# KerkDovan/univer-ocr

Measured on NVIDIA B200. Metric: my_model inference images/sec (page tiles through Monochrome->Paragraph + Line + Char forward), higher is better.
Workload: dtype tf32/f32

## Files before the change

### univer_ocr_b200/csrc/tc_gemm.cu

```cuda
#include <cuda.h>

#include <mutex>

#include "conv_common.cuh"
#include "gemm_common.cuh"
#include "tc_ptx.cuh"

namespace uocr {

typedef CUresult (*EncodeTiledFn)(CUtensorMap*, CUtensorMapDataType, cuuint32_t, void*, const cuuint64_t*,
                                  const cuuint64_t*, const cuuint32_t*, const cuuint32_t*,
                                  CUtensorMapInterleave, CUtensorMapSwizzle, CUtensorMapL2promotion,
                                  CUtensorMapFloatOOBfill);

static EncodeTiledFn encode_tiled() {
    static EncodeTiledFn fn = nullptr;
    static std::once_flag once;
    std::call_once(once, [] {
        void* p = nullptr;
        cudaDriverEntryPointQueryResult q;
        if (cudaGetDriverEntryPoint("cuTensorMapEncodeTiled", &p, cudaEnableDefault, &q) == cudaSuccess &&
            q == cudaDriverEntryPointSuccess)
            fn = reinterpret_cast<EncodeTiledFn>(p);
    });
// ... 603 lines not shown
        const uint64_t da[2] = {(uint64_t)K, (uint64_t)M}, sa[1] = {(uint64_t)lda * 4};
        const uint32_t ba[2] = {TC_BK, TC_BM};
        rc = make_tmap(&ma, A, 2, da, sa, ba);
    }
    if (rc) return rc;
    const uint64_t db[2] = {(uint64_t)K, (uint64_t)N}, sb[1] = {(uint64_t)ldb * 4};
    const uint32_t bb[2] = {TC_BK, (uint32_t)(pair ? p.nt / 2 : p.nt)};
    rc = make_tmap(&mb, Bt, 2, db, sb, bb);
    if (rc) return rc;
    static int num_sms = 0, num_pairs = 0;
    if (!num_sms) {
        int dev = 0;
        cudaGetDevice(&dev);
        cudaDeviceGetAttribute(&num_sms, cudaDevAttrMultiProcessorCount, dev);
        cudaError_t e = cudaFuncSetAttribute(tc_gemm_persistent_kernel<false>, cudaFuncAttributeMaxDynamicSharedMemorySize,
                                             227 * 1024);
        if (e == cudaSuccess)
            e = cudaFuncSetAttribute(tc_gemm_persistent_kernel<true>, cudaFuncAttributeMaxDynamicSharedMemorySize,
                                     227 * 1024);
        if (e != cudaSuccess) { num_sms = 0; set_error("cudaFuncSetAttribute: %s", cudaGetErrorString(e)); return UOCR_ERR_CUDA; }
    }
    const int n_tiles = (int)ceil_div(N, p.nt);
    if (pair) {
        const int m_tiles = (int)ceil_div(M, 2 * TC_BM);
        const int64_t tiles = (int64_t)m_tiles * n_tiles;
        cudaLaunchConfig_t cfg{};
        cudaLaunchAttribute attr[1];
        attr[0].id = cudaLaunchAttributeClusterDimension;
        attr[0].val.clusterDim.x = 2; attr[0].val.clusterDim.y = 1; attr[0].val.clusterDim.z = 1;
        cfg.blockDim = dim3(TCP_THREADS); cfg.dynamicSmemBytes = smem; cfg.stream = st; cfg.attrs = attr; cfg.numAttrs = 1;
        if (!num_pairs) {
            cfg.gridDim = dim3((unsigned)num_sms & ~1u);
            int n = 0;
            if (cudaOccupancyMaxActiveClusters(&n, tc_gemm_persistent_kernel<true>, &cfg) != cudaSuccess || n <= 0) {
                cudaGetLastError();
                n = num_sms / 2;
            }
            num_pairs = n < num_sms / 2 ? n : num_sms / 2;
        }
        cfg.gridDim = dim3(2u * (unsigned)(tiles < num_pairs ? tiles : num_pairs));
        cudaError_t e = cudaLaunchKernelEx(&cfg, tc_gemm_persistent_kernel<true>, ma, mb, p, m_tiles, n_tiles);
        if (e != cudaSuccess) { set_error("cluster launch: %s", cudaGetErrorString(e)); return UOCR_ERR_CUDA; }
        UOCR_LAUNCHED("tc_gemm_persistent_pair_tf32");
        return UOCR_OK;
    }
    const int m_tiles = (int)ceil_div(M, TC_BM);
    const int64_t tiles = (int64_t)m_tiles * n_tiles;
    const unsigned grid = (unsigned)(tiles < num_sms ? tiles : num_sms);
    tc_gemm_persistent_kernel<false><<<grid, TCP_THREADS, smem, st>>>(ma, mb, p, m_tiles, n_tiles);
    UOCR_LAUNCHED("tc_gemm_persistent_tf32");
    return UOCR_OK;
}

int tc_gemm_mn_atomic(const float* At, int64_t lda, const float* B, int64_t ldb, float* C, int64_t ldc,
                      int64_t M, int64_t N, int64_t K, cudaStream_t st) {
    if ((lda % 4) || (ldb % 4) || ((reinterpret_cast<uintptr_t>(At) | reinterpret_cast<uintptr_t>(B)) & 15))
        return UOCR_ERR_UNSUPPORTED;
    if (M <= 0 || N <= 0 || K <= 0 || M > 0x7fffffff || K > 0x7fffffff) return UOCR_ERR_UNSUPPORTED;
    TcParams p{};
    p.C = C; p.ldc = ldc; p.M = M; p.N = N; p.num_kb = (int)ceil_div(K, TC_BK);
    p.nt = N >= 256 ? 256 : (int)(((N + 31) / 32) * 32);
    p.act = UOCR_ACT_NONE; p.atomic = 1;
    const int64_t tiles = ceil_div(M, TC_BM) * ceil_div(N, p.nt);
    int64_t splits = (148 + tiles - 1) / tiles;
    if (splits > p.num_kb / 8) splits = p.num_kb / 8;
    if (splits < 1) splits = 1;
    if (splits > 65535) splits = 65535;
    p.kb_per_split = (int)ceil_div(p.num_kb, splits);
    splits = ceil_div(p.num_kb, p.kb_per_split);
    CUtensorMap ma, mb;
    const uint64_t da[2] = {(uint64_t)M, (uint64_t)K}, sa[1] = {(uint64_t)lda * 4};
    const uint32_t box[2] = {32, TC_BK};
    int rc = make_tmap(&ma, At, 2, da, sa, box, true);
    if (rc) return rc;
    const uint64_t db[2] = {(uint64_t)N, (uint64_t)K}, sb[1] = {(uint64_t)ldb * 4};
    rc = make_tmap(&mb, B, 2, db, sb, box, true);
    if (rc) return rc;
    dim3 grid((unsigned)ceil_div(M, TC_BM), (unsigned)ceil_div(N, p.nt), (unsigned)splits);
    return launch_tc<TC_GEMM_MN>(ma, mb, p, grid, st);
}

__global__ void __launch_bounds__(256) transpose_kernel(const float* __restrict__ src, float* __restrict__ dst,
                                                        int rows, int cols, int64_t src_pitch, int64_t dst_pitch) {
    __shared__ float t[32][33];
    const int c0 = blockIdx.x * 32, r0 = blockIdx.y * 32;
    const int tx = threadIdx.x & 31, ty = threadIdx.x >> 5;
    for (int i = ty; i < 32; i += 8) {
        const int r = r0 + i, c = c0 + tx;
        t[i][tx] = (r < rows && c < cols) ? src[(int64_t)r * src_pitch + c] : 0.f;
    }
    __syncthreads();
    for (int i = ty; i < 32; i += 8) {
        const int c = c0 + i, r = r0 + tx;
        if (c < cols && r < rows) dst[(int64_t)c * dst_pitch + r] = t[tx][i];
    }
}

static int transpose_async(const float* src, float* dst, int rows, int cols, int64_t src_pitch, int64_t dst_pitch,
                           cudaStream_t st) {
    dim3 grid((cols + 31) / 32, (rows + 31) / 32);
    transpose_kernel<<<grid, 256, 0, st>>>(src, dst, rows, cols, src_pitch, dst_pitch);
    UOCR_LAUNCHED("transpose");
    return UOCR_OK;
}

int fc_fwd_fast(int math_mode, const float* x, const float* w, const float* w_kmajor, float* y, int64_t batch,
                int64_t n_in, int64_t n_out, int act, float alpha, cudaStream_t st) {
    if (math_mode != UOCR_MATH_TF32) return UOCR_ERR_UNSUPPORTED;
    if (n_in % 4 || batch < 128 || n_in < 32 || n_out < 16) return UOCR_ERR_UNSUPPORTED;
    if (!encode_tiled()) return UOCR_ERR_UNSUPPORTED;
    Scratch wt(st);
    if (!w_kmajor) {
        int rc = wt.alloc(sizeof(float) * n_out * n_in);
        if (rc) return rc;
        rc = transpose_async(w, (float*)wt.ptr, (int)n_in, (int)n_out, n_out, n_in, st);
        if (rc) return rc;
        w_kmajor = (const float*)wt.ptr;
    }
    return tc_gemm_tn(x, n_in, w_kmajor, n_in, y, n_out, batch, n_out, n_in, w + n_in * n_out, act, alpha, 0, st);
}

int fc_window_fwd_fast(int math_mode, const float* x, const float* w, const float* w_kmajor, float* y, int64_t n,
                       int64_t wd, int64_t c, int width, int64_t n_out, int act, float alpha, cudaStream_t st) {
    const int64_t n_in = (int64_t)width * c, batch = n * wd;
    if (math_mode != UOCR_MATH_TF32 || !encode_tiled()) return UOCR_ERR_UNSUPPORTED;
    if (wd % TC_BM || c % TC_BK || n_out < 128 || n_out % 4 || (reinterpret_cast<uintptr_t>(x) & 15)) return UOCR_ERR_UNSUPPORTED;
    const int64_t nt = n_out >= 256 ? 256 : ((n_out + 15) / 16) * 16;
    if (ceil_div(batch, TC_BM) * ceil_div(n_out, nt) < 96) return UOCR_ERR_UNSUPPORTED;
    Scratch wt(st);
    if (!w_kmajor) {
        int rc = wt.alloc(sizeof(float) * n_out * n_in);
        if (rc) return rc;
        rc = transpose_async(w, (float*)wt.ptr, (int)n_in, (int)n_out, n_out, n_in, st);
        if (rc) return rc;
        w_kmajor = (const float*)wt.ptr;
    }
    const WindowGeom win{n, wd, c, width};
    return tc_gemm_tn_persistent_impl(x, 0, &win, w_kmajor, n_in, y, n_out, batch, n_out, n_in, w + n_in * n_out, act,
                                      alpha, 0, st);
}

int weights_to_kmajor(const float* w, float* wt, int64_t k_rows, int64_t n_cols, cudaStream_t st) {
    if (k_rows > 0x7fffffff || n_cols > 0x7fffffff) return UOCR_ERR_UNSUPPORTED;
    return transpose_async(w, wt, (int)k_rows, (int)n_cols, n_cols, k_rows, st);
}

__global__ void __launch_bounds__(256) colsum_kernel(const float* __restrict__ src, int64_t rows, int cols,
                                                     int64_t rows_per_block, float* __restrict__ out) {
    __shared__ float red[8][33];
    const int c = blockIdx.x * 32 + (threadIdx.x & 31);
    const int ty = threadIdx.x >> 5;
    const int64_t r0 = (int64_t)blockIdx.y * rows_per_block;
    const int64_t r1 = min(rows, r0 + rows_per_block);
    float s0 = 0.f, s1 = 0.f, s2 = 0.f, s3 = 0.f;
    if (c < cols) {
        int64_t r = r0 + ty;
        for (; r + 24 < r1; r += 32) {
            s0 += __ldg(src + r * cols + c);
            s1 += __ldg(src + (r + 8) * cols + c);
            s2 += __ldg(src + (r + 16) * cols + c);
            s3 += __ldg(src + (r + 24) * cols + c);
        }
        for (; r < r1; r += 8) s0 += __ldg(src + r * cols + c);
    }
    red[ty][threadIdx.x & 31] = (s0 + s1) + (s2 + s3);
    __syncthreads();
    if (ty == 0 && c < cols) {
        float t = 0.f;
#pragma unroll
        for (int k = 0; k < 8; ++k) t += red[k][threadIdx.x];
        atomicAdd(out + c, t);
    }
}

static int colsum_async(const float* src, int64_t rows, int cols, float* out, int accumulate, cudaStream_t st) {
    if (!accumulate) {
        cudaError_t e = cudaMemsetAsync(out, 0, sizeof(float) * cols, st);
        if (e != cudaSuccess) { set_error("memset: %s", cudaGetErrorString(e)); return UOCR_ERR_CUDA; }
    }
    const int gx = (cols + 31) / 32;
    int64_t gy = ceil_div(148 * 8, gx);
    const int64_t max_gy = ceil_div(rows, 64);
    if (gy > max_gy) gy = max_gy;
    if (gy < 1) gy = 1;
    if (gy > 65535) gy = 65535;
    const int64_t rpb = ceil_div(rows, gy);
    colsum_kernel<<<dim3((unsigned)gx, (unsigned)ceil_div(rows, rpb)), 256, 0, st>>>(src, rows, cols, rpb, out);
    UOCR_LAUNCHED("colsum");
    return UOCR_OK;
// ... 534 lines not shown
```

### univer_ocr_b200/csrc/hourglass.cu

```cuda
#include "conv_common.cuh"
#include "tc_ptx.cuh"

namespace uocr {

struct HourglassParams {
    const float* x; float* y;
    const float* w[5]; const float* b[5];
    int H, W;
    float alpha;
    int act_end; float alpha_end;
};

constexpr int HG_WSLOT = 28;

template <int TH, int TW>
struct HG {
    static constexpr int XH = TH + 25, XW = TW + 27, XP = (XW + 1 + 3) & ~3, XROWS = XH + 2;
    static constexpr int D1H = TH / 2 + 11, D1W = TW / 2 + 11, D1P = (D1W + 3 + 3) & ~3;
    static constexpr int D2H = TH / 4 + 4, D2W = TW / 4 + 4, D2P = (D2W + 2 + 3 + 3) & ~3;
    static constexpr int U2H = TH / 2 + 4, U2W = TW / 2 + 4, U2P = (U2W + 3 + 3) & ~3;
    static constexpr int U1H = TH + 4, U1W = TW + 4, U1P = (U1W + 3 + 3) & ~3;
    static constexpr int FLOATS = XROWS * XP + D1H * D1P + D2H * D2P + U2H * U2P + 5 * HG_WSLOT + 2 * 36 + 6;
    static_assert(U1H * U1P <= XROWS * XP, "U1 fits into the x block");
};

constexpr int HG_THREADS = 256;
__host__ __device__ constexpr int hg_threads(int th) { return th >= 64 ? 512 : HG_THREADS; }

template <int N4>
__device__ __forceinline__ void hg_load_weights(const float* __restrict__ src, float* w) {
#pragma unroll
    for (int i = 0; i < N4; ++i) {
        const float4 v = reinterpret_cast<const float4*>(src)[i];
        w[4 * i] = v.x; w[4 * i + 1] = v.y; w[4 * i + 2] = v.z; w[4 * i + 3] = v.w;
    }
}

template <int DH, int DW, int DP, int SP, int R, int NT>
__device__ __forceinline__ void hg_down(const float* __restrict__ src, float* __restrict__ dst, const float* __restrict__ wb,
                                        int gy0, int gx0, int hl, int wl, float alpha) {
    float w[28];
    hg_load_weights<7>(wb, w);
    const float bias = w[25];
    constexpr int STRIPS = (DH + R - 1) / R;
    for (int item = threadIdx.x; item < STRIPS * DW; item += NT) {
        const int s = item / DW, c = item - s * DW, r0 = R * s;
        float acc[R];
#pragma unroll
        for (int j = 0; j < R; ++j) acc[j] = bias;
#pragma unroll
        for (int rr = 0; rr < 2 * R + 3; ++rr) {
            const float2* row = reinterpret_cast<const float2*>(src + (2 * r0 + rr) * SP + 2 * c);
            const float2 a = row[0], b = row[1], e = row[2];
            const float in[5] = {a.x, a.y, b.x, b.y, e.x};
#pragma unroll
            for (int j = 0; j < R; ++j) {
                const int ky = rr - 2 * j;
                if (ky >= 0 && ky < 5) {
#pragma unroll
                    for (int kx = 0; kx < 5; ++kx) acc[j] = fmaf(w[ky * 5 + kx], in[kx], acc[j]);
                }
            }
        }
        const bool colin = (unsigned)(gx0 + c) < (unsigned)wl;
#pragma unroll
        for (int j = 0; j < R; ++j) {
            const float v = fmaxf(acc[j], acc[j] * alpha);
            if (r0 + j < DH) dst[(r0 + j) * DP + c] = (colin && (unsigned)(gy0 + r0 + j) < (unsigned)hl) ? v : 0.f;
        }
    }
}

template <int DH, int DW, int DP, int SP, int R, int NT>
__device__ __forceinline__ void hg_down_pairs(const float* __restrict__ src, float* __restrict__ dst, const float* __restrict__ wb,
                                              int gy0, int gx0, int hl, int wl, float alpha) {
    float w[28];
    hg_load_weights<7>(wb, w);
    const float bias = w[25];
    constexpr int STRIPS = (DH + R - 1) / R, PAIRS = DW / 2 + 1;
    for (int item = threadIdx.x; item < STRIPS * PAIRS; item += NT) {
        const int s = item / PAIRS, pr = item - s * PAIRS, r0 = R * s;
        float acc[R][2];
#pragma unroll
        for (int j = 0; j < R; ++j) acc[j][0] = acc[j][1] = bias;
#pragma unroll
        for (int rr = 0; rr < 2 * R + 3; ++rr) {
            const float4* row = reinterpret_cast<const float4*>(src + (2 * r0 + rr) * SP + 4 * pr);
            const float4 u = row[0], v = row[1];
            const float in[8] = {u.x, u.y, u.z, u.w, v.x, v.y, v.z, v.w};
#pragma unroll
            for (int j = 0; j < R; ++j) {
                const int ky = rr - 2 * j;
                if (ky >= 0 && ky < 5) {
#pragma unroll
                    for (int kx = 0; kx < 5; ++kx) {
                        acc[j][0] = fmaf(w[ky * 5 + kx], in[kx], acc[j][0]);
                        acc[j][1] = fmaf(w[ky * 5 + kx], in[2 + kx], acc[j][1]);
                    }
                }
            }
        }
        const int c1 = 2 * pr, c0 = c1 - 1;
        const bool in0 = pr > 0 && (unsigned)(gx0 + c0) < (unsigned)wl, in1 = c1 < DW && (unsigned)(gx0 + c1) < (unsigned)wl;
#pragma unroll
        for (int j = 0; j < R; ++j) {
            if (r0 + j < DH) {
                const bool rowin = (unsigned)(gy0 + r0 + j) < (unsigned)hl;
                const float v0 = fmaxf(acc[j][0], acc[j][0] * alpha), v1 = fmaxf(acc[j][1], acc[j][1] * alpha);
                if (pr > 0) dst[(r0 + j) * DP + c0] = (rowin && in0) ? v0 : 0.f;
                if (c1 < DW) dst[(r0 + j) * DP + c1] = (rowin && in1) ? v1 : 0.f;
            }
        }
    }
}

template <int DH, int DW, int DP, int SP, int NT>
__device__ __forceinline__ void hg_up(const float* __restrict__ src, float* __restrict__ dst, const float* __restrict__ wf,
                                      float bias, int gy0, int gx0, int hl, int wl, float alpha) {
    float w[36];
    hg_load_weights<9>(wf, w);
    constexpr int GROUPS = (DW + 3) / 4;
    for (int item = threadIdx.x; item < (DH / 2) * GROUPS; item += NT) {
        const int j = item / GROUPS, n0 = (item - j * GROUPS) * 2;
        float s[3][4];
#pragma unroll
        for (int a = 0; a < 3; ++a) {
            const float2* row = reinterpret_cast<const float2*>(src + (j + a) * SP + n0);
            const float2 u = row[0], v = row[1];
            s[a][0] = u.x; s[a][1] = u.y; s[a][2] = v.x; s[a][3] = v.y;
        }
#pragma unroll
        for (int py = 0; py < 2; ++py) {
            float o[4];
#pragma unroll
            for (int i = 0; i < 2; ++i)
#pragma unroll
                for (int px = 0; px < 2; ++px) {
                    float acc = bias;
#pragma unroll
                    for (int a = 0; a < 3; ++a)
#pragma unroll
                        for (int b = 0; b < 3; ++b) acc = fmaf(w[((py * 2 + px) * 3 + a) * 3 + b], s[a][i + b], acc);
                    o[2 * i + px] = fmaxf(acc, acc * alpha);
                }
            const bool rowin = (unsigned)(gy0 + 2 * j + py) < (unsigned)hl;
#pragma unroll
            for (int k = 0; k < 4; ++k)
                if (!(rowin && (unsigned)(gx0 + 2 * n0 + k) < (unsigned)wl)) o[k] = 0.f;
            *reinterpret_cast<float4*>(dst + (2 * j + py) * DP + 2 * n0) = make_float4(o[0], o[1], o[2], o[3]);
        }
    }
}

template <int NT>
__device__ __forceinline__ void hg_fold(const float* __restrict__ w25, float* __restrict__ wf) {
    for (int i = threadIdx.x; i < 36; i += NT) {
        const int b = i % 3, a = (i / 3) % 3, px = (i / 9) % 2, py = i / 18;
        const int ylo = py == 0 ? 2 * a : (a == 0 ? 0 : 2 * a - 1), yhi = py == 0 ? min(2 * a + 1, 4) : (a == 0 ? 0 : 2 * a);
        const int xlo = px == 0 ? 2 * b : (b == 0 ? 0 : 2 * b - 1), xhi = px == 0 ? min(2 * b + 1, 4) : (b == 0 ? 0 : 2 * b);
        float s = 0.f;
        for (int ky = ylo; ky <= yhi; ++ky)
            for (int kx = xlo; kx <= xhi; ++kx) s += w25[ky * 5 + kx];
        wf[i] = s;
    }
}

template <int TH, int TW>
__global__ void __launch_bounds__(hg_threads(TH), TH >= 64 ? 2 : 4) hourglass1_fwd_kernel(const HourglassParams p,
                                                                       const __grid_constant__ CUtensorMap map_x) {
    using G = HG<TH, TW>;
    constexpr int NT = hg_threads(TH);
    extern __shared__ __align__(128) float hg_smem[];
    float* sX = hg_smem;
    float* sD1 = sX + G::XROWS * G::XP;
    float* sD2 = sD1 + G::D1H * G::D1P;
    float* sU2 = sD2 + G::D2H * G::D2P;
    float* sU1 = sX;
    float* sW = sU2 + G::U2H * G::U2P;
    float* sF = sW + 5 * HG_WSLOT;

    const int ox0 = blockIdx.x * TW, oy0 = blockIdx.y * TH;
    float* yim = p.y + (int64_t)blockIdx.z * p.H * p.W;
    const int tid = threadIdx.x;

    uint64_t* bar = reinterpret_cast<uint64_t*>(sF + 2 * 36);
    if (tid == 0) {
        mbar_init(smem_u32(bar), 1);
        asm volatile("fence.mbarrier_init.release.cluster;" ::: "memory");
        mbar_arrive_expect_tx(smem_u32(bar), (uint32_t)(G::XH * G::XP * sizeof(float)));
        tma_load_3d(smem_u32(sX), &map_x, smem_u32(bar), ox0 - 16, oy0 - 14, (int)blockIdx.z);
    }
    if (tid < 26) {
#pragma unroll
        for (int l = 0; l < 5; ++l) sW[l * HG_WSLOT + tid] = tid < 25 ? __ldg(p.w[l] + tid) : __ldg(p.b[l]);
    }
    for (int i = tid; i < 2 * G::XP; i += NT) sX[G::XH * G::XP + i] = 0.f;
    __syncthreads();
    mbar_wait(smem_u32(bar), 0);
    hg_fold<NT>(sW + 2 * HG_WSLOT, sF);
    hg_fold<NT>(sW + 3 * HG_WSLOT, sF + 36);
    const int hy0 = oy0 / 2, hx0 = ox0 / 2, qy0 = oy0 / 4, qx0 = ox0 / 4;
    hg_down_pairs<G::D1H, G::D1W, G::D1P, G::XP, 5, NT>(sX, sD1, sW, hy0 - 6, hx0 - 6, p.H / 2, p.W / 2, p.alpha);
    __syncthreads();
    hg_down<G::D2H, G::D2W, G::D2P, G::D1P, (G::D2H % 2 == 0) ? 2 : 4, NT>(sD1, sD2, sW + HG_WSLOT, qy0 - 2, qx0 - 2, p.H / 4, p.W / 4, p.alpha);
    __syncthreads();
    hg_up<G::U2H, G::U2W, G::U2P, G::D2P, NT>(sD2, sU2, sF, sW[2 * HG_WSLOT + 25], hy0 - 2, hx0 - 2, p.H / 2, p.W / 2, p.alpha);
    __syncthreads();
    hg_up<G::U1H, G::U1W, G::U1P, G::U2P, NT>(sU2, sU1, sF + 36, sW[3 * HG_WSLOT + 25], oy0 - 2, ox0 - 2, p.H, p.W, p.alpha);
    __syncthreads();
    {
        float w[28];
        hg_load_weights<7>(sW + 4 * HG_WSLOT, w);
        const float bias = w[25];
        constexpr int GROUPS = TW / 4, RE = 4;
        for (int item = tid; item < (TH / RE) * GROUPS; item += NT) {
            const int r = (item / GROUPS) * RE, c0 = (item - (item / GROUPS) * GROUPS) * 4;
            float acc[RE][4];
#pragma unroll
            for (int k = 0; k < RE; ++k)
#pragma unroll
                for (int j = 0; j < 4; ++j) acc[k][j] = bias;
#pragma unroll
            for (int rr = 0; rr < RE + 4; ++rr) {
                const float4* row = reinterpret_cast<const float4*>(sU1 + (r + rr) * G::U1P + c0);
                const float4 u = row[0], v = row[1];
                const float in[8] = {u.x, u.y, u.z, u.w, v.x, v.y, v.z, v.w};
#pragma unroll
                for (int k = 0; k < RE; ++k) {
                    const int ky = rr - k;
                    if (ky >= 0 && ky < 5) {
#pragma unroll
                        for (int kx = 0; kx < 5; ++kx)
#pragma unroll
                            for (int j = 0; j < 4; ++j) acc[k][j] = fmaf(w[ky * 5 + kx], in[j + kx], acc[k][j]);
                    }
                }
            }
            const int gx = ox0 + c0;
            if (gx < p.W) {
#pragma unroll
                for (int k = 0; k < RE; ++k) {
                    const int gy = oy0 + r + k;
                    if (gy < p.H)
                        *reinterpret_cast<float4*>(yim + (int64_t)gy * p.W + gx) =
                            make_float4(apply_act_fast(acc[k][0], p.act_end, p.alpha_end),
                                        apply_act_fast(acc[k][1], p.act_end, p.alpha_end),
                                        apply_act_fast(acc[k][2], p.act_end, p.alpha_end),
                                        apply_act_fast(acc[k][3], p.act_end, p.alpha_end));
                }
            }
        }
    }
}

static int hourglass1_unsupported() {
    set_error("hourglass1_fwd: unsupported geometry (H, W must be multiples of 4)");
    return UOCR_ERR_UNSUPPORTED;
}

template <int TH>
static int hourglass1_launch(const HourglassParams& p, const float* x, int64_t n, int64_t h, int64_t wd, cudaStream_t st) {
    constexpr int TW = 128;
    using G = HG<TH, TW>;
    const uint64_t dims[3] = {(uint64_t)wd, (uint64_t)h, (uint64_t)n};
    const uint64_t strides[2] = {(uint64_t)wd * 4, (uint64_t)wd * h * 4};
    const uint32_t box[3] = {(uint32_t)G::XP, (uint32_t)G::XH, 1};
    CUtensorMap map{};
    const int rc = make_tmap_plain_f32(&map, x, 3, dims, strides, box);
    if (rc != UOCR_OK) return rc;
    const size_t smem = sizeof(float) * G::FLOATS;
    static bool configured = false;
    if (!configured) {
        cudaError_t e = cudaFuncSetAttribute(hourglass1_fwd_kernel<TH, TW>, cudaFuncAttributeMaxDynamicSharedMemorySize,
                                             (int)smem);
        if (e != cudaSuccess) { set_error("cudaFuncSetAttribute: %s", cudaGetErrorString(e)); return UOCR_ERR_CUDA; }
        configured = true;
    }
    dim3 grid((unsigned)ceil_div(wd, TW), (unsigned)ceil_div(h, TH), (unsigned)n);
    if (grid.y > 65535) return hourglass1_unsupported();
    hourglass1_fwd_kernel<TH, TW><<<grid, hg_threads(TH), smem, st>>>(p, map);
    UOCR_LAUNCHED("hourglass1_fwd");
    return UOCR_OK;
}

int hourglass1_fwd(const float* x, const float* const* w, const float* const* b, float* y, int64_t n, int64_t h,
                   int64_t wd, float alpha, int act_end, float alpha_end, cudaStream_t st) {
    if (h % 4 || wd % 4 || n > 65535 || alpha < 0.f || alpha > 1.f) return hourglass1_unsupported();
    if ((reinterpret_cast<uintptr_t>(x) | reinterpret_cast<uintptr_t>(y)) & 15) return hourglass1_unsupported();
    HourglassParams p{};
    p.x = x; p.y = y;
    for (int l = 0; l < 5; ++l) { p.w[l] = w[l]; p.b[l] = b[l]; }
    p.H = (int)h; p.W = (int)wd; p.alpha = alpha; p.act_end = act_end; p.alpha_end = alpha_end;
    const int64_t blocks64 = n * ceil_div(h, 64) * ceil_div(wd, 128);
    if (blocks64 >= 148 * 2 * 2) return hourglass1_launch<64>(p, x, n, h, wd, st);
    return hourglass1_launch<32>(p, x, n, h, wd, st);
}

}

static int hourglass1_entry(const float* x, const float* const* weights, const float* const* biases, float* y, int64_t n,
                            int64_t h, int64_t w, float alpha, int act_end, float alpha_end, int math_mode, void* stream) {
    using namespace uocr;
    UOCR_REQUIRE(x && y && weights && biases, "NULL pointer");
    for (int l = 0; l < 5; ++l) UOCR_REQUIRE(weights[l] && biases[l], "NULL weight pointer (level %d)", l);
    UOCR_REQUIRE(n > 0 && h > 0 && w > 0 && h < (1 << 30) && w < (1 << 30), "bad dimension");
    UOCR_REQUIRE(act_end >= UOCR_ACT_NONE && act_end <= UOCR_ACT_SIGMOID, "unknown activation %d", act_end);
    UOCR_REQUIRE(math_mode == UOCR_MATH_FP32 || math_mode == UOCR_MATH_TF32, "unknown math mode %d", math_mode);
    return hourglass1_fwd(x, weights, biases, y, n, h, w, alpha, act_end, alpha_end, as_stream(stream));
}

extern "C" int uocr_hourglass1_fwd(const float* x, const float* const* weights, const float* const* biases, float* y,
                                   int64_t n, int64_t h, int64_t w, float alpha, int act_end, float alpha_end,
                                   void* stream) {
    return hourglass1_entry(x, weights, biases, y, n, h, w, alpha, act_end, alpha_end, UOCR_MATH_FP32, stream);
}

extern "C" int uocr_hourglass1_fwd_mode(const float* x, const float* const* weights, const float* const* biases, float* y,
                                        int64_t n, int64_t h, int64_t w, float alpha, int act_end, float alpha_end,
                                        int math_mode, void* stream) {
    return hourglass1_entry(x, weights, biases, y, n, h, w, alpha, act_end, alpha_end, math_mode, stream);
}
```

Baseline: 171,600.

## Add slab-reuse tcgen05 kernel for sliding-window FC layers

After: 173,700 (median of 6 runs). +1.2%, better.

```diff
diff --git a/univer_ocr_b200/csrc/tc_gemm.cu b/univer_ocr_b200/csrc/tc_gemm.cu
--- a/univer_ocr_b200/csrc/tc_gemm.cu
+++ b/univer_ocr_b200/csrc/tc_gemm.cu
@@ -679,6 +679,260 @@
     return UOCR_OK;
 }
 
+constexpr int WFC_CHUNK = 128;
+constexpr uint32_t WFC_HALF_BYTES = WFC_CHUNK * TC_BK * 4;
+
+struct WinFcParams {
+    float* y; int64_t n_out;
+    int m_tiles, n_tiles;
+    int chunks_per_row;
+    int64_t chunks;
+    int tiles_per_line;
+    int cblocks, half, num_kb;
+    int rot_period;
+    int stages;
+    uint32_t slab_bytes, slab_box_bytes;
+    int act; float alpha;
+};
+
+struct WinFcUnits {
+    int64_t q, end;
+    int cpr;
+    __device__ WinFcUnits(const WinFcParams& p)
+        : q(p.chunks * blockIdx.x / gridDim.x), end(p.chunks * (blockIdx.x + 1) / gridDim.x), cpr(p.chunks_per_row) {}
+    __device__ bool next(int& mt, int& col0, int& ncols) {
+        if (q >= end) return false;
+        mt = (int)(q / cpr);
+        const int cq = (int)(q - (int64_t)mt * cpr);
+        const bool two = (cq & 1) == 0 && q + 1 < end;
+        col0 = cq * WFC_CHUNK; ncols = two ? 2 * WFC_CHUNK : WFC_CHUNK;
+        q += two ? 2 : 1;
+        return true;
+    }
+};
+
+__global__ void __launch_bounds__(TCP_THREADS, 1) tc_window_fc_kernel(const __grid_constant__ CUtensorMap map_x,
+                                                                     const __grid_constant__ CUtensorMap map_b,
+                                                                     const float* __restrict__ bias, const WinFcParams p) {
+    extern __shared__ __align__(1024) uint8_t smem_raw[];
+    uint8_t* smem = reinterpret_cast<uint8_t*>((reinterpret_cast<uintptr_t>(smem_raw) + 1023) & ~(uintptr_t)1023);
+    const uint32_t slab_set = (uint32_t)p.cblocks * p.slab_bytes;
+    constexpr uint32_t stage_bytes = 2 * WFC_HALF_BYTES;
+    uint8_t* slab = smem;
+    uint8_t* ring = smem + 2 * slab_set;
+    float* s_bias = reinterpret_cast<float*>(ring + (size_t)p.stages * stage_bytes);
+    float* s_stage = s_bias + p.n_out;
+    uint64_t* bars = reinterpret_cast<uint64_t*>(s_stage + 8 * 512);
+    uint64_t* full = bars;
+    uint64_t* empty = bars + p.stages;
+    uint64_t* tmem_full = bars + 2 * p.stages;
+    uint64_t* tmem_empty = bars + 2 * p.stages + 2;
+    uint64_t* slab_full = bars + 2 * p.stages + 4;
+    uint64_t* slab_empty = bars + 2 * p.stages + 6;
+    uint32_t* tmem_slot = reinterpret_cast<uint32_t*>(bars + 2 * p.stages + 8);
+
+    const int warp = threadIdx.x >> 5, lane = threadIdx.x & 31;
+    for (int i = threadIdx.x; i < p.n_out; i += TCP_THREADS) s_bias[i] = bias ? __ldg(bias + i) : 0.f;
+    if (threadIdx.x == 0) {
+        for (int s = 0; s < p.stages; ++s) {
+            mbar_init(smem_u32(&full[s]), 1);
+            mbar_init(smem_u32(&empty[s]), 1);
+        }
+        for (int b = 0; b < 2; ++b) {
+            mbar_init(smem_u32(&tmem_full[b]), 1);
+            mbar_init(smem_u32(&tmem_empty[b]), 8);
+            mbar_init(smem_u32(&slab_full[b]), 1);
+            mbar_init(smem_u32(&slab_empty[b]), 1);
+        }
+        asm volatile("fence.mbarrier_init.release.cluster;" ::: "memory");
+    }
+    if (warp == 1) {
+        asm volatile("tcgen05.alloc.cta_group::1.sync.aligned.shared::cta.b32 [%0], %1;"
+                     ::"r"(smem_u32(tmem_slot)), "r"(4 * WFC_CHUNK) : "memory");
+        asm volatile("tcgen05.relinquish_alloc_permit.cta_group::1.sync.aligned;" ::: "memory");
+    }
+    tc_fence_before();
+    __syncthreads();
+    tc_fence_after();
+    const uint32_t tmem_base = *tmem_slot;
+    auto first_kb = [&](int mt, int col0) {
+        return p.rot_period ? (int)(((int64_t)mt * p.n_tiles + col0 / (2 * WFC_CHUNK)) % p.rot_period) % p.num_kb : 0;
+    };
+
+    if (warp == 0) {
+        if (lane == 0) {
+            WinFcUnits units(p);
+            int it = 0, r = -1, cur = -1, mt, col0, ncols;
+            while (units.next(mt, col0, ncols)) {
+                if (mt != cur) {
+                    cur = mt; ++r;
+                    const int buf = r & 1;
+                    const int line = mt / p.tiles_per_line, wx0 = (mt - line * p.tiles_per_line) * TC_BM;
+                    mbar_wait(smem_u32(&slab_empty[buf]), ((r >> 1) & 1) ^ 1);
+                    mbar_arrive_expect_tx(smem_u32(&slab_full[buf]), (uint32_t)p.cblocks * p.slab_box_bytes);
+                    for (int cb = 0; cb < p.cblocks; ++cb)
+                        tma_load_3d(smem_u32(slab + buf * slab_set + cb * p.slab_bytes), &map_x,
+                                    smem_u32(&slab_full[buf]), cb * TC_BK, wx0 - p.half, line);
+                }
+                const int rot = first_kb(mt, col0);
+                for (int kb = 0; kb < p.num_kb; ++kb, ++it) {
+                    const int s = it % p.stages;
+                    mbar_wait(smem_u32(&empty[s]), ((it / p.stages) & 1) ^ 1);
+                    const int kbr = kb + rot >= p.num_kb ? kb + rot - p.num_kb : kb + rot;
+                    const uint32_t sb = smem_u32(ring + s * stage_bytes);
+                    mbar_arrive_expect_tx(smem_u32(&full[s]), (uint32_t)ncols * TC_BK * 4);
+                    for (int h = 0; h < ncols; h += WFC_CHUNK)
+                        tma_load_2d(sb + (uint32_t)h * TC_BK * 4, &map_b, smem_u32(&full[s]), kbr * TC_BK, col0 + h);
+                }
+            }
+        }
+    } else if (warp == 1) {
+        if (lane == 0) {
+            const uint32_t idesc0 = (1u << 4) | (2u << 7) | (2u << 10) | ((uint32_t)(TC_BM >> 4) << 24);
+            WinFcUnits units(p);
+            int it = 0, t = 0, r = -1, cur = -1, mt, col0, ncols;
+            uint32_t slab0 = 0;
+            while (units.next(mt, col0, ncols)) {
+                if (mt != cur) {
+                    if (r >= 0) tc_commit(smem_u32(&slab_empty[r & 1]));
+                    cur = mt; ++r;
+                    mbar_wait(smem_u32(&slab_full[r & 1]), (r >> 1) & 1);
+                    tc_fence_after();
+                    slab0 = smem_u32(slab + (r & 1) * slab_set);
+                }
+                const int acc = t & 1;
+                mbar_wait(smem_u32(&tmem_empty[acc]), ((t >> 1) & 1) ^ 1);
+                tc_fence_after();
+                const uint32_t tacc = tmem_base + (uint32_t)(acc * 2 * WFC_CHUNK);
+                const uint32_t idesc = idesc0 | ((uint32_t)(ncols >> 3) << 17);
+                const int rot = first_kb(mt, col0);
+                for (int kb = 0; kb < p.num_kb; ++kb, ++it) {
+                    const int s = it % p.stages;
+                    mbar_wait(smem_u32(&full[s]), (it / p.stages) & 1);
+                    tc_fence_after();
+                    const int kbr = kb + rot >= p.num_kb ? kb + rot - p.num_kb : kb + rot;
+                    const int k = kbr / p.cblocks, cb = kbr - k * p.cblocks;
+                    const uint64_t da = make_kmajor_sw128_desc(slab0 + (uint32_t)cb * p.slab_bytes + (uint32_t)k * 128u);
+                    const uint64_t db = make_kmajor_sw128_desc(smem_u32(ring + s * stage_bytes));
+#pragma unroll
+                    for (int kk = 0; kk < TC_BK / 8; ++kk)
+                        tc_mma_tf32(tacc, da + (uint64_t)(kk * 2), db + (uint64_t)(kk * 2), idesc,
+                                    (kb > 0 || kk > 0) ? 1u : 0u);
+                    tc_commit(smem_u32(&empty[s]));
+                }
+                tc_commit(smem_u32(&tmem_full[acc]));
+                ++t;
+            }
+        }
+    } else {
+        const int e = warp - 2, q = warp & 3, half = e >> 2;
+        float4* stg = reinterpret_cast<float4*>(s_stage) + e * 128;
+        const int sub_r = lane >> 2, sub_g = lane & 3;
+        WinFcUnits units(p);
+        int t = 0, mt, col0, ncols;
+        while (units.next(mt, col0, ncols)) {
+            const int acc = t & 1;
+            const int nhc = ncols >> 4;
+            float* yrow = p.y + ((int64_t)mt * TC_BM + q * 32) * p.n_out;
+            mbar_wait(smem_u32(&tmem_full[acc]), (t >> 1) & 1);
+            tc_fence_after();
+            const uint32_t tq = tmem_base + ((uint32_t)(q * 32) << 16) + (uint32_t)(acc * 2 * WFC_CHUNK);
+            uint32_t va[16], vb[16];
+            auto handle = [&](uint32_t* cur, uint32_t* nxt, int hc) {
+                tc_wait_ld();
+                if (hc + 2 < nhc) {
+                    tc_ld16_nowait(tq + (uint32_t)((hc + 2) * 16), nxt);
+                } else {
+                    tc_fence_before();
+                    if (lane == 0) mbar_arrive(smem_u32(&tmem_empty[acc]));
+                }
+                const int c = col0 + hc * 16;
+                const float4* bs = reinterpret_cast<const float4*>(s_bias + c);
+                __syncwarp();
+#pragma unroll
+                for (int g = 0; g < 4; ++g) {
+                    const float4 b4 = bs[g];
+                    stg[lane * 4 + (g ^ ((lane >> 1) & 3))] =
+                        make_float4(apply_act_fast(__uint_as_float(cur[4 * g]) + b4.x, p.act, p.alpha),
+                                    apply_act_fast(__uint_as_float(cur[4 * g + 1]) + b4.y, p.act, p.alpha),
+                                    apply_act_fast(__uint_as_float(cur[4 * g + 2]) + b4.z, p.act, p.alpha),
+                                    apply_act_fast(__uint_as_float(cur[4 * g + 3]) + b4.w, p.act, p.alpha));
+                }
+                __syncwarp();
+#pragma unroll
+                for (int i = 0; i < 4; ++i) {
+                    const int rr = 8 * i + sub_r;
+                    *reinterpret_cast<float4*>(yrow + rr * p.n_out + c + 4 * sub_g) =
+                        stg[rr * 4 + (sub_g ^ ((rr >> 1) & 3))];
+                }
+            };
+            tc_ld16_nowait(tq + (uint32_t)(half * 16), va);
+            for (int hc = half; hc < nhc; hc += 4) {
+                handle(va, vb, hc);
+                handle(vb, va, hc + 2);
+            }
+            ++t;
+        }
+    }
+
+    tc_fence_before();
+    __syncthreads();
+    if (warp == 1) {
+        tc_fence_after();
+        asm volatile("tcgen05.dealloc.cta_group::1.sync.aligned.b32 %0, %1;" ::"r"(tmem_base), "r"(4 * WFC_CHUNK) : "memory");
+    }
+}
+
+static int window_fc_slab(const float* x, const float* wt, const float* bias, float* y, int64_t n, int64_t wd, int64_t c,
+                          int width, int64_t n_out, int act, float alpha, cudaStream_t st) {
+    const int64_t m_tiles = n * wd / TC_BM;
+    if (n_out % (2 * WFC_CHUNK) || n_out > 2048 || (reinterpret_cast<uintptr_t>(y) & 15)) return UOCR_ERR_UNSUPPORTED;
+    if (TC_BM + width - 1 > 256 || m_tiles > 0x7fffffff) return UOCR_ERR_UNSUPPORTED;
+    WinFcParams p{};
+    p.y = y; p.n_out = n_out;
+    p.m_tiles = (int)m_tiles; p.n_tiles = (int)(n_out / (2 * WFC_CHUNK));
+    p.chunks_per_row = (int)(n_out / WFC_CHUNK); p.chunks = m_tiles * p.chunks_per_row;
+    p.tiles_per_line = (int)(wd / TC_BM);
+    p.cblocks = (int)(c / TC_BK); p.half = width / 2; p.num_kb = width * p.cblocks;
+    p.act = act; p.alpha = alpha;
+    const uint32_t box_rows = TC_BM + width - 1;
+    p.slab_box_bytes = box_rows * 128u;
+    p.slab_bytes = (p.slab_box_bytes + 1023u) & ~1023u;
+    const size_t stage_bytes = 2 * WFC_HALF_BYTES;
+    const size_t fixed = 1024  + 2 * (size_t)p.cblocks * p.slab_bytes + (size_t)n_out * 4 + 8 * 2048 + 8 * 8 + 16;
+    const size_t max_smem = 227 * 1024;
+    if (fixed + 2 * (stage_bytes + 16) > max_smem) return UOCR_ERR_UNSUPPORTED;
+    p.stages = (int)((max_smem - fixed) / (stage_bytes + 16));
+    if (p.stages > 8) p.stages = 8;
+    const size_t smem = fixed + (size_t)p.stages * (stage_bytes + 16);
+    static int num_sms = 0;
+    if (!num_sms) {
+        int dev = 0, sms = 0;
+        cudaGetDevice(&dev);
+        cudaDeviceGetAttribute(&sms, cudaDevAttrMultiProcessorCount, dev);
+        cudaError_t e = cudaFuncSetAttribute(tc_window_fc_kernel, cudaFuncAttributeMaxDynamicSharedMemorySize, (int)max_smem);
+        if (e != cudaSuccess) { set_error("cudaFuncSetAttribute: %s", cudaGetErrorString(e)); return UOCR_ERR_CUDA; }
+        num_sms = sms;
+    }
+    const int64_t tiles = m_tiles * p.n_tiles;
+    p.rot_period = tiles >= 96 ? (int)(tiles < num_sms ? tiles : num_sms) : 0;
+    CUtensorMap mx, mb;
+    const uint64_t dx[3] = {(uint64_t)c, (uint64_t)wd, (uint64_t)n};
+    const uint64_t sx[2] = {(uint64_t)c * 4, (uint64_t)wd * c * 4};
+    const uint32_t bx[3] = {TC_BK, box_rows, 1};
+    int rc = make_tmap(&mx, x, 3, dx, sx, bx);
+    if (rc) return rc;
+    const int64_t n_in = (int64_t)width * c;
+    const uint64_t db[2] = {(uint64_t)n_in, (uint64_t)n_out}, sb[1] = {(uint64_t)n_in * 4};
+    const uint32_t bb[2] = {TC_BK, WFC_CHUNK};
+    rc = make_tmap(&mb, wt, 2, db, sb, bb);
+    if (rc) return rc;
+    const unsigned grid = (unsigned)(p.chunks < num_sms ? p.chunks : num_sms);
+    tc_window_fc_kernel<<<grid, TCP_THREADS, smem, st>>>(mx, mb, bias, p);
+    UOCR_LAUNCHED("tc_window_fc_tf32");
+    return UOCR_OK;
+}
+
 int tc_gemm_mn_atomic(const float* At, int64_t lda, const float* B, int64_t ldb, float* C, int64_t ldc,
                       int64_t M, int64_t N, int64_t K, cudaStream_t st) {
     if ((lda % 4) || (ldb % 4) || ((reinterpret_cast<uintptr_t>(At) | reinterpret_cast<uintptr_t>(B)) & 15))
@@ -753,7 +1007,8 @@
     if (math_mode != UOCR_MATH_TF32 || !encode_tiled()) return UOCR_ERR_UNSUPPORTED;
     if (wd % TC_BM || c % TC_BK || n_out < 128 || n_out % 4 || (reinterpret_cast<uintptr_t>(x) & 15)) return UOCR_ERR_UNSUPPORTED;
     const int64_t nt = n_out >= 256 ? 256 : ((n_out + 15) / 16) * 16;
-    if (ceil_div(batch, TC_BM) * ceil_div(n_out, nt) < 96) return UOCR_ERR_UNSUPPORTED;
+    const bool many_tiles = ceil_div(batch, TC_BM) * ceil_div(n_out, nt) >= 96;
+    if (n_out % (2 * WFC_CHUNK) && !many_tiles) return UOCR_ERR_UNSUPPORTED;
     Scratch wt(st);
     if (!w_kmajor) {
         int rc = wt.alloc(sizeof(float) * n_out * n_in);
@@ -762,6 +1017,8 @@
         if (rc) return rc;
         w_kmajor = (const float*)wt.ptr;
     }
+    const int rc = window_fc_slab(x, w_kmajor, w + n_in * n_out, y, n, wd, c, width, n_out, act, alpha, st);
+    if (rc != UOCR_ERR_UNSUPPORTED || !many_tiles) return rc;
     const WindowGeom win{n, wd, c, width};
     return tc_gemm_tn_persistent_impl(x, 0, &win, w_kmajor, n_in, y, n_out, batch, n_out, n_in, w + n_in * n_out, act,
                                       alpha, 0, st);
```

## Add persistent vertical-sweep hourglass kernel reusing halo rows across bands

Applied to the files above, without the earlier changes.

Result: faster. 171,300 before, 174,800 after, median of 6 (+2.0%).

```diff
diff --git a/univer_ocr_b200/csrc/hourglass.cu b/univer_ocr_b200/csrc/hourglass.cu
--- a/univer_ocr_b200/csrc/hourglass.cu
+++ b/univer_ocr_b200/csrc/hourglass.cu
@@ -25,7 +25,6 @@
 };
 
 constexpr int HG_THREADS = 256;
-__host__ __device__ constexpr int hg_threads(int th) { return th >= 64 ? 512 : HG_THREADS; }
 
 template <int N4>
 __device__ __forceinline__ void hg_load_weights(const float* __restrict__ src, float* w) {
@@ -37,13 +36,13 @@
 }
 
 template <int DH, int DW, int DP, int SP, int R, int NT>
-__device__ __forceinline__ void hg_down(const float* __restrict__ src, float* __restrict__ dst, const float* __restrict__ wb,
+__device__ __forceinline__ void hg_down(int tid, const float* __restrict__ src, float* __restrict__ dst, const float* __restrict__ wb,
                                         int gy0, int gx0, int hl, int wl, float alpha) {
     float w[28];
     hg_load_weights<7>(wb, w);
     const float bias = w[25];
     constexpr int STRIPS = (DH + R - 1) / R;
-    for (int item = threadIdx.x; item < STRIPS * DW; item += NT) {
+    for (int item = tid; item < STRIPS * DW; item += NT) {
         const int s = item / DW, c = item - s * DW, r0 = R * s;
         float acc[R];
 #pragma unroll
@@ -72,13 +71,13 @@
 }
 
 template <int DH, int DW, int DP, int SP, int R, int NT>
-__device__ __forceinline__ void hg_down_pairs(const float* __restrict__ src, float* __restrict__ dst, const float* __restrict__ wb,
+__device__ __forceinline__ void hg_down_pairs(int tid, const float* __restrict__ src, float* __restrict__ dst, const float* __restrict__ wb,
                                               int gy0, int gx0, int hl, int wl, float alpha) {
     float w[28];
     hg_load_weights<7>(wb, w);
     const float bias = w[25];
     constexpr int STRIPS = (DH + R - 1) / R, PAIRS = DW / 2 + 1;
-    for (int item = threadIdx.x; item < STRIPS * PAIRS; item += NT) {
+    for (int item = tid; item < STRIPS * PAIRS; item += NT) {
         const int s = item / PAIRS, pr = item - s * PAIRS, r0 = R * s;
         float acc[R][2];
 #pragma unroll
@@ -115,12 +114,12 @@
 }
 
 template <int DH, int DW, int DP, int SP, int NT>
-__device__ __forceinline__ void hg_up(const float* __restrict__ src, float* __restrict__ dst, const float* __restrict__ wf,
+__device__ __forceinline__ void hg_up(int tid, const float* __restrict__ src, float* __restrict__ dst, const float* __restrict__ wf,
                                       float bias, int gy0, int gx0, int hl, int wl, float alpha) {
     float w[36];
     hg_load_weights<9>(wf, w);
     constexpr int GROUPS = (DW + 3) / 4;
-    for (int item = threadIdx.x; item < (DH / 2) * GROUPS; item += NT) {
+    for (int item = tid; item < (DH / 2) * GROUPS; item += NT) {
         const int j = item / GROUPS, n0 = (item - j * GROUPS) * 2;
         float s[3][4];
 #pragma unroll
@@ -165,11 +164,57 @@
     }
 }
 
+template <int TH, int TW, int U1P, int NT>
+__device__ __forceinline__ void hg_end(int tid, const float* __restrict__ sU1, const float* __restrict__ wb, float* __restrict__ yim,
+                                       int oy0, int ox0, const HourglassParams& p) {
+    float w[28];
+    hg_load_weights<7>(wb, w);
+    const float bias = w[25];
+    constexpr int GROUPS = TW / 4, RE = 4;
+    for (int item = tid; item < (TH / RE) * GROUPS; item += NT) {
+        const int r = (item / GROUPS) * RE, c0 = (item - (item / GROUPS) * GROUPS) * 4;
+        float acc[RE][4];
+#pragma unroll
+        for (int k = 0; k < RE; ++k)
+#pragma unroll
+            for (int j = 0; j < 4; ++j) acc[k][j] = bias;
+#pragma unroll
+        for (int rr = 0; rr < RE + 4; ++rr) {
+            const float4* row = reinterpret_cast<const float4*>(sU1 + (r + rr) * U1P + c0);
+            const float4 u = row[0], v = row[1];
+            const float in[8] = {u.x, u.y, u.z, u.w, v.x, v.y, v.z, v.w};
+#pragma unroll
+            for (int k = 0; k < RE; ++k) {
+                const int ky = rr - k;
+                if (ky >= 0 && ky < 5) {
+#pragma unroll
+                    for (int kx = 0; kx < 5; ++kx)
+#pragma unroll
+                        for (int j = 0; j < 4; ++j) acc[k][j] = fmaf(w[ky * 5 + kx], in[j + kx], acc[k][j]);
+                }
+            }
+        }
+        const int gx = ox0 + c0;
+        if (gx < p.W) {
+#pragma unroll
+            for (int k = 0; k < RE; ++k) {
+                const int gy = oy0 + r + k;
+                if (gy < p.H)
+                    *reinterpret_cast<float4*>(yim + (int64_t)gy * p.W + gx) =
+                        make_float4(apply_act_fast(acc[k][0], p.act_end, p.alpha_end),
+                                    apply_act_fast(acc[k][1], p.act_end, p.alpha_end),
+                                    apply_act_fast(acc[k][2], p.act_end, p.alpha_end),
+                                    apply_act_fast(acc[k][3], p.act_end, p.alpha_end));
+            }
+        }
+    }
+}
+
 template <int TH, int TW>
-__global__ void __launch_bounds__(hg_threads(TH), TH >= 64 ? 2 : 4) hourglass1_fwd_kernel(const HourglassParams p,
+__global__ void __launch_bounds__(HG_THREADS, 4) hourglass1_fwd_kernel(const HourglassParams p,
                                                                        const __grid_constant__ CUtensorMap map_x) {
     using G = HG<TH, TW>;
-    constexpr int NT = hg_threads(TH);
+    constexpr int NT = HG_THREADS;
     extern __shared__ __align__(128) float hg_smem[];
     float* sX = hg_smem;
     float* sD1 = sX + G::XROWS * G::XP;
@@ -200,55 +245,139 @@
     hg_fold<NT>(sW + 2 * HG_WSLOT, sF);
     hg_fold<NT>(sW + 3 * HG_WSLOT, sF + 36);
     const int hy0 = oy0 / 2, hx0 = ox0 / 2, qy0 = oy0 / 4, qx0 = ox0 / 4;
-    hg_down_pairs<G::D1H, G::D1W, G::D1P, G::XP, 5, NT>(sX, sD1, sW, hy0 - 6, hx0 - 6, p.H / 2, p.W / 2, p.alpha);
-    __syncthreads();
-    hg_down<G::D2H, G::D2W, G::D2P, G::D1P, (G::D2H % 2 == 0) ? 2 : 4, NT>(sD1, sD2, sW + HG_WSLOT, qy0 - 2, qx0 - 2, p.H / 4, p.W / 4, p.alpha);
-    __syncthreads();
-    hg_up<G::U2H, G::U2W, G::U2P, G::D2P, NT>(sD2, sU2, sF, sW[2 * HG_WSLOT + 25], hy0 - 2, hx0 - 2, p.H / 2, p.W / 2, p.alpha);
-    __syncthreads();
-    hg_up<G::U1H, G::U1W, G::U1P, G::U2P, NT>(sU2, sU1, sF + 36, sW[3 * HG_WSLOT + 25], oy0 - 2, ox0 - 2, p.H, p.W, p.alpha);
-    __syncthreads();
-    {
-        float w[28];
-        hg_load_weights<7>(sW + 4 * HG_WSLOT, w);
-        const float bias = w[25];
-        constexpr int GROUPS = TW / 4, RE = 4;
-        for (int item = tid; item < (TH / RE) * GROUPS; item += NT) {
-            const int r = (item / GROUPS) * RE, c0 = (item - (item / GROUPS) * GROUPS) * 4;
-            float acc[RE][4];
-#pragma unroll
-            for (int k = 0; k < RE; ++k)
-#pragma unroll
-                for (int j = 0; j < 4; ++j) acc[k][j] = bias;
-#pragma unroll
-            for (int rr = 0; rr < RE + 4; ++rr) {
-                const float4* row = reinterpret_cast<const float4*>(sU1 + (r + rr) * G::U1P + c0);
-                const float4 u = row[0], v = row[1];
-                const float in[8] = {u.x, u.y, u.z, u.w, v.x, v.y, v.z, v.w};
-#pragma unroll
-                for (int k = 0; k < RE; ++k) {
-                    const int ky = rr - k;
-                    if (ky >= 0 && ky < 5) {
-#pragma unroll
-                        for (int kx = 0; kx < 5; ++kx)
-#pragma unroll
-                            for (int j = 0; j < 4; ++j) acc[k][j] = fmaf(w[ky * 5 + kx], in[j + kx], acc[k][j]);
-                    }
-                }
-            }
-            const int gx = ox0 + c0;
-            if (gx < p.W) {
-#pragma unroll
-                for (int k = 0; k < RE; ++k) {
-                    const int gy = oy0 + r + k;
-                    if (gy < p.H)
-                        *reinterpret_cast<float4*>(yim + (int64_t)gy * p.W + gx) =
-                            make_float4(apply_act_fast(acc[k][0], p.act_end, p.alpha_end),
-                                        apply_act_fast(acc[k][1], p.act_end, p.alpha_end),
-                                        apply_act_fast(acc[k][2], p.act_end, p.alpha_end),
-                                        apply_act_fast(acc[k][3], p.act_end, p.alpha_end));
-                }
-            }
+    hg_down_pairs<G::D1H, G::D1W, G::D1P, G::XP, 5, NT>(tid, sX, sD1, sW, hy0 - 6, hx0 - 6, p.H / 2, p.W / 2, p.alpha);
+    __syncthreads();
+    hg_down<G::D2H, G::D2W, G::D2P, G::D1P, (G::D2H % 2 == 0) ? 2 : 4, NT>(tid, sD1, sD2, sW + HG_WSLOT, qy0 - 2, qx0 - 2, p.H / 4, p.W / 4, p.alpha);
+    __syncthreads();
+    hg_up<G::U2H, G::U2W, G::U2P, G::D2P, NT>(tid, sD2, sU2, sF, sW[2 * HG_WSLOT + 25], hy0 - 2, hx0 - 2, p.H / 2, p.W / 2, p.alpha);
+    __syncthreads();
+    hg_up<G::U1H, G::U1W, G::U1P, G::U2P, NT>(tid, sU2, sU1, sF + 36, sW[3 * HG_WSLOT + 25], oy0 - 2, ox0 - 2, p.H, p.W, p.alpha);
+    __syncthreads();
+    hg_end<TH, TW, G::U1P, NT>(tid, sU1, sW + 4 * HG_WSLOT, yim, oy0, ox0, p);
+}
+
+struct HGS {
+    using G = HG<64, 128>;
+    static constexpr int TH = 64, TW = 128, NT = 512;
+    static constexpr int XOFF = (32 - (3 * G::XP) % 32) % 32;
+    static constexpr int U1ROW = 3 + TH;
+    static constexpr int X_OFF = XOFF, U1_OFF = X_OFF + U1ROW * G::XP, D1_OFF = U1_OFF + G::U1H * G::U1P,
+                         D2_OFF = D1_OFF + G::D1H * G::D1P, U2_OFF = D2_OFF + G::D2H * G::D2P,
+                         W_OFF = U2_OFF + G::U2H * G::U2P, F_OFF = W_OFF + 5 * HG_WSLOT, BAR_OFF = F_OFF + 2 * 36;
+    static constexpr int FLOATS = BAR_OFF + 2;
+    static constexpr int XREAD = 3 + 2 * 5 * ((G::D1H + 4) / 5 - 1) + 13;
+    static_assert(XREAD * G::XP <= U1_OFF - X_OFF + G::U1H * G::U1P, "first-band over-read stays inside the allocation");
+    static_assert((X_OFF + 3 * G::XP) % 32 == 0 && U1_OFF % 4 == 0 && D1_OFF % 4 == 0 && D2_OFF % 4 == 0 &&
+                  U2_OFF % 4 == 0 && W_OFF % 4 == 0 && BAR_OFF % 2 == 0, "aligned blocks");
+};
+
+template <int P>
+__device__ __forceinline__ void hg_keep(int tid, float* blk, int from, int n) {
+    float4* d = reinterpret_cast<float4*>(blk);
+    const float4* s = reinterpret_cast<const float4*>(blk + from * P);
+    for (int i = tid; i < n * P / 4; i += HGS::NT) d[i] = s[i];
+}
+
+template <bool FIRST>
+__device__ __forceinline__ void hg_sweep_band(float* sm, const HourglassParams& p, const CUtensorMap* map_next, int oy0,
+                                              int ox0, int z, bool more) {
+    using G = HGS::G;
+    constexpr int NT = HGS::NT, XP = G::XP;
+    int tid;
+    asm volatile("mov.u32 %0, %%tid.x;" : "=r"(tid));
+    float* sX = sm + HGS::X_OFF;
+    float* sU1 = sm + HGS::U1_OFF;
+    float* sD1 = sm + HGS::D1_OFF;
+    float* sD2 = sm + HGS::D2_OFF;
+    float* sU2 = sm + HGS::U2_OFF;
+    const float* sW = sm + HGS::W_OFF;
+    const float* sF = sm + HGS::F_OFF;
+    const int hy0 = oy0 / 2, hx0 = ox0 / 2, qy0 = oy0 / 4, qx0 = ox0 / 4;
+    constexpr int XR = FIRST ? 3 + G::XH : 3 + HGS::TH, D1R = FIRST ? G::D1H : 3 + 32, D2R = FIRST ? G::D2H : 2 + 16,
+                  U2R = FIRST ? G::U2H : 2 + 32;
+    if (FIRST) {
+        hg_down_pairs<G::D1H, G::D1W, G::D1P, XP, 5, NT>(tid, sX + 3 * XP, sD1, sW, hy0 - 6, hx0 - 6, p.H / 2, p.W / 2, p.alpha);
+    } else {
+        hg_keep<G::U1P>(tid, sU1, G::U1H - 4, 4);
+        hg_down_pairs<32, G::D1W, G::D1P, XP, 4, NT>(tid, sX, sD1 + 3 * G::D1P, sW, hy0 + 5, hx0 - 6, p.H / 2, p.W / 2, p.alpha);
+    }
+    __syncthreads();
+    if (FIRST)
+        hg_down<G::D2H, G::D2W, G::D2P, G::D1P, 2, NT>(tid, sD1, sD2, sW + HG_WSLOT, qy0 - 2, qx0 - 2, p.H / 4, p.W / 4, p.alpha);
+    else
+        hg_down<16, G::D2W, G::D2P, G::D1P, 2, NT>(tid, sD1, sD2 + 2 * G::D2P, sW + HG_WSLOT, qy0 + 2, qx0 - 2, p.H / 4, p.W / 4,
+                                                   p.alpha);
+    hg_keep<XP>(tid, sX, XR - 3, 3);
+    __syncthreads();
+    if (more && tid == 0) {
+        asm volatile("fence.proxy.async.shared::cta;" ::: "memory");
+        uint64_t* bar = reinterpret_cast<uint64_t*>(sm + HGS::BAR_OFF);
+        mbar_arrive_expect_tx(smem_u32(bar), (uint32_t)(HGS::TH * XP * sizeof(float)));
+        tma_load_3d(smem_u32(sX + 3 * XP), map_next, smem_u32(bar), ox0 - 16, oy0 + HGS::TH + 11, z);
+    }
+    if (FIRST)
+        hg_up<G::U2H, G::U2W, G::U2P, G::D2P, NT>(tid, sD2, sU2, sF, sW[2 * HG_WSLOT + 25], hy0 - 2, hx0 - 2, p.H / 2, p.W / 2,
+                                                   p.alpha);
+    else
+        hg_up<32, G::U2W, G::U2P, G::D2P, NT>(tid, sD2, sU2 + 2 * G::U2P, sF, sW[2 * HG_WSLOT + 25], hy0 + 2, hx0 - 2, p.H / 2,
+                                              p.W / 2, p.alpha);
+    hg_keep<G::D1P>(tid, sD1, D1R - 3, 3);
+    __syncthreads();
+    if (FIRST)
+        hg_up<G::U1H, G::U1W, G::U1P, G::U2P, NT>(tid, sU2, sU1, sF + 36, sW[3 * HG_WSLOT + 25], oy0 - 2, ox0 - 2, p.H, p.W,
+                                                   p.alpha);
+    else
+        hg_up<HGS::TH, G::U1W, G::U1P, G::U2P, NT>(tid, sU2, sU1 + 4 * G::U1P, sF + 36, sW[3 * HG_WSLOT + 25], oy0 + 2, ox0 - 2,
+                                                    p.H, p.W, p.alpha);
+    hg_keep<G::D2P>(tid, sD2, D2R - 2, 2);
+    __syncthreads();
+    hg_end<HGS::TH, HGS::TW, G::U1P, NT>(tid, sU1, sW + 4 * HG_WSLOT, p.y + (int64_t)z * p.H * p.W, oy0, ox0, p);
+    hg_keep<G::U2P>(tid, sU2, U2R - 2, 2);
+    __syncthreads();
+}
+
+__global__ void __launch_bounds__(HGS::NT, 2) hourglass1_sweep_kernel(const HourglassParams p,
+                                                                      const __grid_constant__ CUtensorMap map_first,
+                                                                      const __grid_constant__ CUtensorMap map_next,
+                                                                      int n, int strips, int bands) {
+    using G = HGS::G;
+    extern __shared__ __align__(128) float hg_smem[];
+    const int tid = threadIdx.x;
+    float* sX = hg_smem + HGS::X_OFF;
+    float* sW = hg_smem + HGS::W_OFF;
+    uint64_t* bar = reinterpret_cast<uint64_t*>(hg_smem + HGS::BAR_OFF);
+    if (tid == 0) {
+        mbar_init(smem_u32(bar), 1);
+        asm volatile("fence.mbarrier_init.release.cluster;" ::: "memory");
+    }
+    if (tid < 26) {
+#pragma unroll
+        for (int l = 0; l < 5; ++l) sW[l * HG_WSLOT + tid] = tid < 25 ? __ldg(p.w[l] + tid) : __ldg(p.b[l]);
+    }
+    for (int i = tid; i < (HGS::XREAD - 3 - G::XH) * G::XP; i += HGS::NT) sX[(3 + G::XH) * G::XP + i] = 0.f;
+    __syncthreads();
+    hg_fold<HGS::NT>(sW + 2 * HG_WSLOT, hg_smem + HGS::F_OFF);
+    hg_fold<HGS::NT>(sW + 3 * HG_WSLOT, hg_smem + HGS::F_OFF + 36);
+
+    const int total = n * strips * bands;
+    const int b0 = (int)((int64_t)blockIdx.x * total / gridDim.x), b1 = (int)((int64_t)(blockIdx.x + 1) * total / gridDim.x);
+    int band = b0 % bands, s = (b0 / bands) % strips, z = b0 / (bands * strips);
+    uint32_t phase = 0;
+    for (int b = b0; b < b1; ++b) {
+        const int oy0 = band * HGS::TH, ox0 = s * HGS::TW;
+        const bool first = b == b0 || band == 0, more = b + 1 < b1 && band + 1 < bands;
+        if (first && tid == 0) {
+            asm volatile("fence.proxy.async.shared::cta;" ::: "memory");
+            mbar_arrive_expect_tx(smem_u32(bar), (uint32_t)(G::XH * G::XP * sizeof(float)));
+            tma_load_3d(smem_u32(sX + 3 * G::XP), &map_first, smem_u32(bar), ox0 - 16, oy0 - 14, z);
+        }
+        mbar_wait(smem_u32(bar), phase);
+        phase ^= 1;
+        if (first) hg_sweep_band<true>(hg_smem, p, &map_next, oy0, ox0, z, more);
+        else hg_sweep_band<false>(hg_smem, p, &map_next, oy0, ox0, z, more);
+        if (++band == bands) {
+            band = 0;
+            if (++s == strips) { s = 0; ++z; }
         }
     }
 }
@@ -258,15 +387,19 @@
     return UOCR_ERR_UNSUPPORTED;
 }
 
-template <int TH>
-static int hourglass1_launch(const HourglassParams& p, const float* x, int64_t n, int64_t h, int64_t wd, cudaStream_t st) {
-    constexpr int TW = 128;
-    using G = HG<TH, TW>;
+static int hourglass1_tmap(CUtensorMap* map, const float* x, int64_t n, int64_t h, int64_t wd, int box_rows) {
     const uint64_t dims[3] = {(uint64_t)wd, (uint64_t)h, (uint64_t)n};
     const uint64_t strides[2] = {(uint64_t)wd * 4, (uint64_t)wd * h * 4};
-    const uint32_t box[3] = {(uint32_t)G::XP, (uint32_t)G::XH, 1};
+    const uint32_t box[3] = {(uint32_t)HG<32, 128>::XP, (uint32_t)box_rows, 1};
+    return make_tmap_plain_f32(map, x, 3, dims, strides, box);
+}
+
+static int hourglass1_launch_blocks(const HourglassParams& p, const float* x, int64_t n, int64_t h, int64_t wd,
+                                    cudaStream_t st) {
+    constexpr int TH = 32, TW = 128;
+    using G = HG<TH, TW>;
     CUtensorMap map{};
-    const int rc = make_tmap_plain_f32(&map, x, 3, dims, strides, box);
+    const int rc = hourglass1_tmap(&map, x, n, h, wd, G::XH);
     if (rc != UOCR_OK) return rc;
     const size_t smem = sizeof(float) * G::FLOATS;
     static bool configured = false;
@@ -278,7 +411,34 @@
     }
     dim3 grid((unsigned)ceil_div(wd, TW), (unsigned)ceil_div(h, TH), (unsigned)n);
     if (grid.y > 65535) return hourglass1_unsupported();
-    hourglass1_fwd_kernel<TH, TW><<<grid, hg_threads(TH), smem, st>>>(p, map);
+    hourglass1_fwd_kernel<TH, TW><<<grid, HG_THREADS, smem, st>>>(p, map);
+    UOCR_LAUNCHED("hourglass1_fwd");
+    return UOCR_OK;
+}
+
+static int hourglass1_launch_sweep(const HourglassParams& p, const float* x, int64_t n, int64_t h, int64_t wd,
+                                   cudaStream_t st) {
+    CUtensorMap map_first{}, map_next{};
+    int rc = hourglass1_tmap(&map_first, x, n, h, wd, HGS::G::XH);
+    if (rc == UOCR_OK) rc = hourglass1_tmap(&map_next, x, n, h, wd, HGS::TH);
+    if (rc != UOCR_OK) return rc;
+    const size_t smem = sizeof(float) * HGS::FLOATS;
+    static int resident = 0;
+    if (!resident) {
+        int dev = 0, sms = 0, per_sm = 0;
+        cudaError_t e = cudaFuncSetAttribute(hourglass1_sweep_kernel, cudaFuncAttributeMaxDynamicSharedMemorySize, (int)smem);
+        if (e == cudaSuccess) e = cudaGetDevice(&dev);
+        if (e == cudaSuccess) e = cudaDeviceGetAttribute(&sms, cudaDevAttrMultiProcessorCount, dev);
+        if (e == cudaSuccess) e = cudaOccupancyMaxActiveBlocksPerMultiprocessor(&per_sm, hourglass1_sweep_kernel, HGS::NT, smem);
+        if (e != cudaSuccess) { set_error("hourglass1 sweep setup: %s", cudaGetErrorString(e)); return UOCR_ERR_CUDA; }
+        if (per_sm < 1) { set_error("hourglass1 sweep: kernel does not fit an SM"); return UOCR_ERR_CUDA; }
+        resident = sms * per_sm;
+    }
+    const int strips = (int)ceil_div(wd, HGS::TW), bands = (int)ceil_div(h, HGS::TH);
+    const int64_t total = n * strips * bands;
+    if (total > INT32_MAX) return hourglass1_unsupported();
+    const unsigned grid = (unsigned)(total < resident ? total : resident);
+    hourglass1_sweep_kernel<<<grid, HGS::NT, smem, st>>>(p, map_first, map_next, (int)n, strips, bands);
     UOCR_LAUNCHED("hourglass1_fwd");
     return UOCR_OK;
 }
@@ -291,9 +451,9 @@
     p.x = x; p.y = y;
     for (int l = 0; l < 5; ++l) { p.w[l] = w[l]; p.b[l] = b[l]; }
     p.H = (int)h; p.W = (int)wd; p.alpha = alpha; p.act_end = act_end; p.alpha_end = alpha_end;
-    const int64_t blocks64 = n * ceil_div(h, 64) * ceil_div(wd, 128);
-    if (blocks64 >= 148 * 2 * 2) return hourglass1_launch<64>(p, x, n, h, wd, st);
-    return hourglass1_launch<32>(p, x, n, h, wd, st);
+    const int64_t bands = n * ceil_div(h, 64) * ceil_div(wd, 128);
+    if (bands >= 148 * 2 * 2) return hourglass1_launch_sweep(p, x, n, h, wd, st);
+    return hourglass1_launch_blocks(p, x, n, h, wd, st);
 }
 
 }
```
